# google-research/se3ds

Hardware: AMD Instinct MI355X
Metric: panoramas/sec (G+D train step) at 512x1024 RGB-D (higher is better)
Workload: dtype bf16; 1 GPU; configs/highres 512x1024 full GAN step train_g_d (G+D+hinge+depth+wc losses, clip, Adam, EMA), ResNet-101 gen_dims 128, per-GPU batch 8, d_step_per_g_step 1; per_gpu_batch=8, global_batch=8, parallelism=dp1

## Files before the change

### include/se3ds_hip.h

```cpp
#ifndef SE3DS_HIP_H_
#define SE3DS_HIP_H_

#include <stddef.h>
#include <stdint.h>

#ifdef __cplusplus
extern "C" {
#endif

#define SE3DS_OK 0
#define SE3DS_E_BADSHAPE (-1)
#define SE3DS_E_BADDTYPE (-2)
#define SE3DS_E_WORKSPACE (-3)
#define SE3DS_E_LAUNCH (-4)
#define SE3DS_E_UNSUPPORTED (-5)

#define SE3DS_F32 0
#define SE3DS_I32 1
#define SE3DS_U8 2
#define SE3DS_BF16 3
#define SE3DS_FEAT_BYTE_RANGE 0x100
#define SE3DS_XYZ1_ONES_PRESET 0x200

const char* se3ds_version(void);
// ... 198 lines not shown
                         int c, const float* mean, const float* rstd, int act, float alpha,
                         float* sums, float* dbeta_out, float* dgamma_out, const void* act_mask,
                         void* workspace, size_t workspace_bytes, void* stream);
int se3ds_norm_bwd_apply(const void* dy, const void* y, const void* x, int dtype, int g, int64_t r,
                         int c, const float* mean, const float* rstd, const float* gamma,
                         const float* sums, float count, int act, float alpha, void* dx,
                         void* dres, const void* act_mask, int in_act, float in_alpha,
                         void* stream);
int se3ds_norm_bwd_apply_rows(const void* dy, const void* x, int dtype, int64_t r, int c,
                              const float* mean, const float* rstd, const float* gamma,
                              const float* sums, float count, int act, float alpha, void* dx,
                              void* dres, const void* act_mask, const float* sum_row,
                              const float* out_row, float* colsum_dst, void* workspace,
                              size_t workspace_bytes, void* stream);
int se3ds_norm_bwd_cg_supported(int dtype, int64_t r, int c, int act, int has_mask, int in_act);
size_t se3ds_norm_bwd_cg_workspace_bytes(int c);
int se3ds_norm_bwd_cg_col_rows(int64_t r, int c);
int se3ds_norm_bwd_cg(const void* dy, const void* x, int dtype, int64_t r, int c, const float* mean,
                      const float* rstd, const float* gamma, float count, int act, float alpha,
                      void* dx, void* dres, const void* act_mask, int in_act, float in_alpha,
                      float* dbeta_out, float* dgamma_out, float* sums_out, const float* sum_row,
                      const float* out_row, float* colpart, void* workspace, size_t workspace_bytes,
                      void* stream);
int se3ds_affine_bwd(const void* dy, const void* y, int dtype, int g, int64_t r, int c,
                     const float* scale, int act, float alpha, void* dx, void* dres,
                     const void* act_mask, void* stream);

int se3ds_act_bwd(const void* dy, const void* y, int dtype, int64_t n, int act, float alpha,
                  void* dx, void* stream);
int se3ds_add(const void* a, const void* b, int dtype, int64_t n, void* out, void* stream);
int se3ds_row_scale(const void* x, int dtype, int64_t rows, int c, const float* scale, void* out,
                    void* stream);
int se3ds_maxpool2x2_fwd(const void* x, int dtype, int n, int h, int w, int c, void* y,
                         void* stream);
int se3ds_maxpool2x2_bwd(const void* dy, const void* x, const void* y, int dtype, int n, int h,
                         int w, int c, void* dx, void* stream);
int se3ds_avgpool3s2_fwd(const void* x, int dtype, int n, int h, int w, int c, void* y,
                         void* stream);
int se3ds_avgpool3s2_bwd(const void* dy, int dtype, int n, int h, int w, int c, void* dx,
                         void* stream);
int se3ds_upsample2x_fwd(const void* x, int dtype, int n, int h, int w, int c, void* y,
                         void* stream);
int se3ds_upsample2x_bwd(const void* dy, int dtype, int n, int h, int w, int c, void* dx,
                         void* stream);
int se3ds_copy_channels(const void* src, int src_dtype, int src_c, int src_c0, void* dst,
                        int dst_dtype, int dst_c, int dst_c0, int ncopy, int64_t rows,
// ... 266 lines not shown
```

### se3ds_amd/csrc/norm.hip

```cpp
#include "common.h"
#include <type_traits>
#include <cstdlib>

namespace se3ds {
namespace {

struct Layout2D {
  int cx;
  int ry;
  int vec;
  int ctiles;
};
inline Layout2D make_layout(int C, int V) {
  Layout2D l;
  l.vec = (C % V == 0) ? V : 1;
  int cvec = C / l.vec;
  int cx = 1;
  while (cx < cvec && cx < 256) cx <<= 1;
  l.cx = cx;
  l.ry = 256 / cx;
  l.ctiles = (int)ceil_div(cvec, cx);
  return l;
}

// ... 156 lines not shown
    red2[k][q][ch] = v;
    __syncthreads();
    if (t < 128) {
      const int kk = t >> 6;
      const int c = blockIdx.y * 64 + ch;
      if (c < C)
        partial[(((int64_t)g * rblocks + blockIdx.x) * 2 + kk) * C + c] = (float)(red2[kk][0][ch] + red2[kk][1][ch]);
    }
    return;
  }
  if (ty == 0 && cok) {
    for (int t = 1; t < ry; ++t) {
#pragma unroll
      for (int e = 0; e < VEC; ++e) {
        s0[e] += red[0][(t * cx + tx) * VEC + e];
        s1[e] += red[1][(t * cx + tx) * VEC + e];
      }
    }
    float* P = partial + (((int64_t)g * rblocks + blockIdx.x) * 2) * C;
#pragma unroll
    for (int e = 0; e < VEC; ++e) {
      P[c0 + e] = (float)s0[e];
      P[C + c0 + e] = (float)s1[e];
    }
  }
}

template <int COLS, int LANES>
__global__ void __launch_bounds__(256)
norm_final_reduce_kernel(const float* __restrict__ partial, int rblocks, int C, int G,
                         float* __restrict__ sums, float* __restrict__ dst0,
                         float* __restrict__ dst1) {
  static_assert(COLS * LANES == 256, "block shape");
  __shared__ double sh[LANES][COLS + 1];
  const int g = blockIdx.y;
  const int cl = threadIdx.x % COLS;
  const int col = blockIdx.x * COLS + cl;
  const int lane_b = threadIdx.x / COLS;
  double s0 = 0, s1 = 0, s2 = 0, s3 = 0;
  if (col < 2 * C) {
    const float* P = partial + (int64_t)g * rblocks * 2 * C + col;
    int b = lane_b;
    for (; b + 3 * LANES < rblocks; b += 4 * LANES) {
      s0 += P[(int64_t)b * 2 * C];
      s1 += P[(int64_t)(b + LANES) * 2 * C];
      s2 += P[(int64_t)(b + 2 * LANES) * 2 * C];
// ... 185 lines not shown
  VT<float>::load(shift + (int64_t)g * C + c0, reinterpret_cast<float(&)[4]>(sh[0]));
  VT<float>::load(shift + (int64_t)g * C + c0 + 4, reinterpret_cast<float(&)[4]>(sh[4]));
  for (int64_t r = (int64_t)blockIdx.x * ry + ty; r < R; r += (int64_t)gridDim.x * ry) {
    const int64_t off = ((int64_t)g * R + r) * C + c0;
    float xv[VEC], rv[VEC], o[VEC];
    VT<T>::load(x + off, xv);
    if (HAS_RES) VT<T>::load(res + off, rv);
    unsigned bits = 0;
#pragma unroll
    for (int e = 0; e < VEC; ++e) {
      float v = xv[e] * sc[e] + sh[e];
      if (HAS_RES) v += rv[e];
      if (ACT == 1) v = v > 0.f ? v : 0.f;
      if (ACT == 2) v = v > 0.f ? v : v * alpha;
      o[e] = v;
      const uint16_t hb = f32_to_bf16(v);
      bits |= ((hb & 0x7fffu) != 0 && (hb & 0x8000u) == 0) ? (1u << e) : 0u;
    }
    VT<T>::store(y + off, o);
    if (amask) amask[off >> 3] = (uint8_t)bits;
  }
}

template <typename T, int VEC>
__global__ void __launch_bounds__(256)
norm_bwd_apply_kernel(const T* __restrict__ dy, const T* __restrict__ y, const T* __restrict__ x,
                      const float* __restrict__ mean, const float* __restrict__ rstd,
                      const float* __restrict__ gamma, const float* __restrict__ sums, float count,
                      int64_t R, int C, int cx, int ry, int act, float alpha, T* __restrict__ dx,
                      T* __restrict__ dres, const uint8_t* __restrict__ amask, int in_act,
                      float in_alpha) {
  const int g = blockIdx.z;
  const int tx = threadIdx.x % cx, ty = threadIdx.x / cx;
  const int c0 = (blockIdx.y * cx + tx) * VEC;
  if (c0 >= C) return;
  float gr[VEC], k1[VEC], c0k[VEC];
  const float inv_count = 1.0f / count;
#pragma unroll
  for (int e = 0; e < VEC; ++e) {
    const int64_t gc = (int64_t)g * C + c0 + e;
    const float mu = mean[gc], rs = rstd[gc];
    gr[e] = (gamma ? gamma[c0 + e] : 1.0f) * rs;
    const float s0 = sums[((int64_t)g * 2) * C + c0 + e] * inv_count;
    const float s1 = sums[((int64_t)g * 2 + 1) * C + c0 + e] * inv_count;
    k1[e] = gr[e] * rs * s1;
    c0k[e] = mu * k1[e] - gr[e] * s0;
// ... 180 lines not shown
  if (ROWS) {
    float* red = lds_buf;
#pragma unroll
    for (int e = 0; e < VEC; ++e) red[threadIdx.x * VEC + e] = bsum[e];
    __syncthreads();
    if (PRO) {
      if (threadIdx.x < 64) {
        float t = 0.f;
#pragma unroll 8
        for (int q = 0; q < 32; ++q) t += red[q * 64 + threadIdx.x];
        colpart[(int64_t)blockIdx.x * C + blockIdx.y * 64 + threadIdx.x] = t;
      }
    } else
    if (ty == 0 && live) {
      const int ny = 256 / cx;
      float* row = colpart + (int64_t)blockIdx.x * 2 * C + c0;
#pragma unroll
      for (int e = 0; e < VEC; ++e) {
        float t = 0.f;
        for (int q = 0; q < ny; ++q) t += red[(q * cx + tx) * VEC + e];
        row[e] = t;
        row[C + e] = 0.f;
      }
    }
  }
}

template <typename T, int VEC>
__global__ void __launch_bounds__(256)
affine_bwd_kernel(const T* __restrict__ dy, const T* __restrict__ y,
                  const float* __restrict__ scale, int64_t R, int C, int cx, int ry, int act,
                  float alpha, T* __restrict__ dx, T* __restrict__ dres,
                  const uint8_t* __restrict__ amask) {
  const int g = blockIdx.z;
  const int tx = threadIdx.x % cx, ty = threadIdx.x / cx;
  const int c0 = (blockIdx.y * cx + tx) * VEC;
  if (c0 >= C) return;
  float sc[VEC];
#pragma unroll
  for (int e = 0; e < VEC; ++e) sc[e] = scale[(int64_t)g * C + c0 + e];
  for (int64_t r = (int64_t)blockIdx.x * ry + ty; r < R; r += (int64_t)gridDim.x * ry) {
    const int64_t off = ((int64_t)g * R + r) * C + c0;
    float dv[VEC], yv[VEC], o[VEC], dr[VEC];
    const bool use_mask = VEC == 8 && amask != nullptr;
    unsigned mbits = 0;
    if constexpr (VEC > 1) {
// ... 350 lines not shown
#define LAUNCH_ST(AC)                                                                             \
  hipLaunchKernelGGL((norm_partial_kernel<uint16_t, 8, 1, true, AC, true>), gs, dim3(256), 0, s, A,  \
                     (const uint16_t*)nullptr, X, mean, rstd, (const float*)nullptr, r, c, 8, 32,    \
                     act, alpha, rb, part, (const uint8_t*)act_mask)
  if (act == 0) LAUNCH_ST(0); else if (act == 1) LAUNCH_ST(1); else LAUNCH_ST(2);
#undef LAUNCH_ST
  const dim3 ga((unsigned)cg_apply_blocks(r, c), (unsigned)(c / 64), 1);
#define LAUNCH_AP(AC, IA, RW)                                                                     \
  hipLaunchKernelGGL((norm_bwd_apply_fast_kernel<AC, IA, RW, true>), ga, dim3(256), 0, s, A, X, mean, \
                     rstd, gamma, part, count, r, c, 8, 32, alpha, (uint16_t*)dx, (uint16_t*)dres,     \
                     (const uint8_t*)act_mask, in_alpha, sum_row, out_row, colpart, rb, dbeta_out,     \
                     dgamma_out, sums_out)
  if (rows) {
    if (act == 0) LAUNCH_AP(0, 0, true); else if (act == 1) LAUNCH_AP(1, 0, true); else LAUNCH_AP(2, 0, true);
  } else if (in_act == 0) {
    if (act == 0) LAUNCH_AP(0, 0, false); else if (act == 1) LAUNCH_AP(1, 0, false); else LAUNCH_AP(2, 0, false);
  } else {
    if (act == 0) LAUNCH_AP(0, 2, false); else if (act == 1) LAUNCH_AP(1, 2, false); else LAUNCH_AP(2, 2, false);
  }
#undef LAUNCH_AP
  return check_launch("norm_bwd_cg");
}

int se3ds_affine_bwd(const void* dy, const void* y, int dtype, int g, int64_t r, int c,
                     const float* scale, int act, float alpha, void* dx, void* dres,
                     const void* act_mask, void* stream) {
  if (g <= 0 || r <= 0 || c <= 0) return SE3DS_E_BADSHAPE;
  hipStream_t s = as_stream(stream);
#define LAUNCH_AFF(T, V)                                                                      \
  hipLaunchKernelGGL((affine_bwd_kernel<T, V>), ew_grid(l, r, g), dim3(256), 0, s,            \
                     (const T*)dy, (const T*)y, scale, r, c, l.cx, l.ry, act, alpha, (T*)dx,  \
                     (T*)dres, (const uint8_t*)act_mask)
  if (dtype == SE3DS_F32) {
    Layout2D l = make_layout(c, 4);
    if (l.vec > 1) LAUNCH_AFF(float, 4); else LAUNCH_AFF(float, 1);
  } else if (dtype == SE3DS_BF16) {
    Layout2D l = make_layout(c, 8);
    if (l.vec > 1) LAUNCH_AFF(uint16_t, 8); else LAUNCH_AFF(uint16_t, 1);
  } else {
    return SE3DS_E_BADDTYPE;
  }
#undef LAUNCH_AFF
  return check_launch("affine_bwd");
}

}
// ... 1 lines not shown
```

### se3ds_amd/hipops/nn.py

```python
import math
import threading
from collections import namedtuple
from types import SimpleNamespace
from typing import List, Optional

import numpy as np
import os

import torch
import torch.distributed as dist

from se3ds_amd import _lib

ACT_NONE, ACT_RELU, ACT_LRELU = 0, 1, 2
BN_EPS, BN_MOMENTUM = 1e-3, 0.99
IN_EPS = 1e-3


def _L():
  return _lib.lib()


def _all_reduce_sum(t, group, kind):
  from se3ds_amd.trainers import dist_utils
# ... 1112 lines not shown
    ctx.record(bwd)
  return out


class NormLayer:

  def __init__(self, store: ParamStore, name, c, kind='batch'):
    self.store, self.name, self.c, self.kind = store, name, c, kind
    store.add(name + '/gamma', (c,), ones_init)
    store.add(name + '/beta', (c,), zeros_init)
    if kind == 'batch':
      store.add(name + '/moving_mean', (c,), zeros_init, trainable=False)
      store.add(name + '/moving_variance', (c,), ones_init, trainable=False)
    self._cg_colpart = None


_NORM_DEBUG = {} if os.environ.get('SE3DS_NORM_DEBUG') else None
_FUSED_BN_BWD = os.environ.get('SE3DS_FUSED_BN_BWD', '0') == '1'
_FUSED_ROW_SCALE = os.environ.get('SE3DS_FUSED_ROW_SCALE', '1') != '0'
_NORM_CG = os.environ.get('SE3DS_NORM_CG', '1') != '0'
_CONVT_2X2 = os.environ.get('SE3DS_CONVT_2X2', '1') != '0'
_MASK_CACHE = os.environ.get('SE3DS_MASK_CACHE', '1') != '0'
_DROP_1X1_MASK = os.environ.get('SE3DS_DROP_1X1_MASK', '1') != '0'


def _norm_debug(who, xd, layer):
  if _NORM_DEBUG is not None:
    key = (who, tuple(xd.shape), layer.kind)
    _NORM_DEBUG[key] = _NORM_DEBUG.get(key, 0) + 1


def _norm_stats(ctx, x, layer, g, r, c, use_moving):
  st, L, inst = layer.store, _L(), layer.kind == 'instance'
  scale = torch.empty((g, c), dtype=torch.float32, device=ctx.device)
  shift, mean, rstd = torch.empty_like(scale), torch.empty_like(scale), torch.empty_like(scale)
  count = float(r)
  affine = (st[layer.name + '/gamma'].data_ptr(), st[layer.name + '/beta'].data_ptr(),
            IN_EPS if inst else BN_EPS, BN_MOMENTUM)
  mm = st[layer.name + '/moving_mean'] if not inst else None
  mv = st[layer.name + '/moving_variance'] if not inst else None
  outs = (scale.data_ptr(), shift.data_ptr(), mean.data_ptr(), rstd.data_ptr(), _lib.stream())
  fused = x.col_stats
  fused = fused if fused is not None and not inst and fused.shape[2] == c else None
  if use_moving:
    _chk(L.se3ds_norm_finalize(None, 1.0, g, c, *affine, mm.data_ptr(), mv.data_ptr(), 1, *outs),
         'se3ds_norm_finalize')
# ... 2 lines not shown
                                           mm.data_ptr(), mv.data_ptr(), *outs),
         'se3ds_norm_reduce_rows_finalize')
    x.col_stats = None
  else:
    if fused is not None:
      sums = torch.empty((1, 2, c), dtype=torch.float32, device=ctx.device)
      ws = ctx.ws('norm', L.se3ds_norm_workspace_bytes(max(1, (fused.shape[0] + 511) // 512), c))
      _chk(L.se3ds_norm_reduce_rows(fused.data_ptr(), fused.shape[0], c, sums.data_ptr(),
                                    ws.data_ptr(), ws.numel(), _lib.stream()),
           'se3ds_norm_reduce_rows')
      x.col_stats = None
    else:
      _norm_debug(layer.name, x.data, layer)
      sums = _colsum(ctx, x.data.data_ptr(), ctx.code, r, c, groups=g)
    if not inst and ctx.world > 1:
      ctx.allreduce_sum(sums)
      count = float(r * ctx.world)
    _chk(L.se3ds_norm_finalize(sums.data_ptr(), count, g, c, *affine, _lib.ptr(mm), _lib.ptr(mv), 0,
                               *outs), 'se3ds_norm_finalize')
  return scale, shift, mean, rstd, count


def norm_act(ctx: Ctx, x: Var, layer: NormLayer, act=ACT_NONE, alpha=0.0, res: Var = None,
             post: Var = None, in_act=None) -> Var:
  xd, inst = x.data, layer.kind == 'instance'
  n, h, w, c = xd.shape
  g, r = (n, h * w) if inst else (1, n * h * w)
  use_moving = (not inst) and (not ctx.training or ctx.bn_use_moving)
  scale, shift, mean, rstd, count = _norm_stats(ctx, x, layer, g, r, c, use_moving)
  y = ctx.empty(xd.shape)
  amask = None
  if (ctx.tape is not None and act != ACT_NONE and post is None and c % 8 == 0 and
      xd.dtype == torch.bfloat16):
    amask = torch.empty(xd.numel() // 8, dtype=torch.uint8, device=ctx.device)
  _chk(_L().se3ds_norm_apply(xd.data_ptr(), ctx.code, g, r, c, scale.data_ptr(), shift.data_ptr(),
                             _lib.ptr(res.data if res is not None else None),
                             _lib.ptr(post.data if post is not None else None), act, float(alpha),
                             y.data_ptr(), _lib.ptr(amask), _lib.stream()), 'se3ds_norm_apply')
  out = Var(y)
  if act != ACT_NONE and ctx.act_taps is not None:
    ctx.act_taps[layer.name] = y
  if (ctx.tape is not None and not inst and not use_moving and post is None and c % 8 == 0 and
      xd.dtype == torch.bfloat16 and (act == ACT_NONE or amask is not None)):
    out.bn_src = BnSrc(xd, amask, mean, rstd, act, alpha)
  sync_bwd = (not inst) and ctx.world > 1 and not use_moving
  if ctx.tape is not None:
    sv = SimpleNamespace(ctx=ctx, x=x, out=out, layer=layer, res=res, post=post, act=act,
                         alpha=float(alpha), in_act=in_act, amask=amask, scale=scale, mean=mean,
                         rstd=rstd, gamma=layer.store[layer.name + '/gamma'], count=count, g=g, r=r,
                         c=c, use_moving=use_moving, sync_bwd=sync_bwd)
    ctx.record(lambda: _norm_bwd(sv), sync=sync_bwd)
  return out


def _norm_bwd(sv):
  ctx, out, xd, c, L = sv.ctx, sv.out, sv.x.data, sv.c, _L()
  dy = out.grad
  fused = out.take_bn_stats()
  out.grad = None
  if dy is None:
    if sv.sync_bwd:
      ctx.allreduce_then(torch.zeros((sv.g, 2, c), dtype=torch.float32, device=ctx.device),
                         lambda: None)
    return
  if sv.post is not None:
    raise NotImplementedError
  lim = ctx.batch_limit
  g, shape = sv.g, xd.shape
  if lim is not None and lim < xd.shape[0]:
    assert sv.layer.kind == 'instance' and dy.shape[0] == lim and not ctx.param_grads
    g, shape = lim, (lim,) + tuple(xd.shape[1:])
  ws = ctx.ws('norm', L.se3ds_norm_workspace_bytes(g, c))
  dres = ctx.empty(shape) if sv.res is not None and sv.res.requires_grad else None
  dx = ctx.empty(shape)
  if sv.use_moving:
    _norm_bwd_moving(sv, dy, dx, dres, g, ws)
  elif (_NORM_CG and not sv.sync_bwd and g == 1 and fused is None and lim is None and
        L.se3ds_norm_bwd_cg_supported(ctx.code, sv.r, c, sv.act, 1 if sv.amask is not None else 0,
                                      sv.in_act[0] if sv.in_act else 0)):
    _norm_bwd_cg(sv, dy, dx, dres)
  else:
    _norm_bwd_split(sv, dy, dx, dres, g, ws, fused, lim)


def _norm_deliver(sv, dx, dres, pre_act, scaled=False):
  if pre_act:
    sv.x.grad_pre_act = True
  accumulate(sv.x, dx)
  if scaled:
    sv.x.grad_scaled = sv.x.gver
  if dres is not None:
    accumulate(sv.res, dres)


# ... 43 lines not shown
  if use_rows:
    nrows = int(L.se3ds_norm_bwd_cg_col_rows(r, c))
    colpart = layer._cg_colpart
    if colpart is None or colpart.numel() < nrows * c:
      colpart = layer._cg_colpart = torch.empty(nrows * c, dtype=torch.float32, device=ctx.device)
  gv, pg = layer.store.grad_views, ctx.param_grads
  in_a, in_alpha = sv.in_act or (0, 0.0)
  _chk(L.se3ds_norm_bwd_cg(
      dy.data_ptr(), x.data.data_ptr(), ctx.code, r, c, sv.mean.data_ptr(), sv.rstd.data_ptr(),
      sv.gamma.data_ptr(), sv.count, sv.act, sv.alpha, dx.data_ptr(), _lib.ptr(dres),
      _lib.ptr(sv.amask), in_a, float(in_alpha),
      gv[layer.name + '/beta'].data_ptr() if pg else None,
      gv[layer.name + '/gamma'].data_ptr() if pg else None, None,
      sink.bias_scale.data_ptr() if use_rows else None,
      sink.out_scale.data_ptr() if use_rows else None, _lib.ptr(colpart), cws.data_ptr(),
      cws.numel(), _lib.stream()), 'se3ds_norm_bwd_cg')
  _norm_debug('cg', x.data, layer)
  if use_rows:
    _norm_debug('fused-rows', x.data, layer)
    reduce_or_defer(ctx, (colpart.data_ptr(), nrows, c // 4, sink.bias_grad().data_ptr()))
  _norm_deliver(sv, dx, dres, bool(sv.in_act), scaled=use_rows)


def _norm_bwd_split(sv, dy, dx, dres, g, ws, fused, lim):
  ctx, x, xd, c, L = sv.ctx, sv.x, sv.x.data, sv.c, _L()
  bs = _norm_bwd_sums(sv, dy, g, ws, fused)
  shared = (sv.r, c, sv.mean.data_ptr(), sv.rstd.data_ptr(), sv.gamma.data_ptr(), bs.data_ptr(),
            sv.count, sv.act, sv.alpha, dx.data_ptr(), _lib.ptr(dres), _lib.ptr(sv.amask))

  def finish():
    sink, rc = x.row_sink, -5
    if (sink is not None and _FUSED_ROW_SCALE and ctx.param_grads and g == 1 and not sv.in_act and
        x.grad is None and lim is None and xd.dtype == torch.bfloat16):
      cws = ctx.ws('norm_rows', L.se3ds_norm_workspace_bytes(3, c))
      rc = L.se3ds_norm_bwd_apply_rows(
          dy.data_ptr(), xd.data_ptr(), ctx.code, *shared, sink.bias_scale.data_ptr(),
          sink.out_scale.data_ptr(), sink.bias_grad().data_ptr(), cws.data_ptr(), cws.numel(),
          _lib.stream())
      if rc == 0:
        _norm_debug('fused-rows', xd, sv.layer)
      elif rc not in (-5, -3):
        _chk(rc, 'se3ds_norm_bwd_apply_rows')
    if rc != 0:
      in_a, in_alpha = sv.in_act or (0, 0.0)
      _chk(L.se3ds_norm_bwd_apply(dy.data_ptr(), sv.out.data.data_ptr(), xd.data_ptr(), ctx.code,
                                  g, *shared, in_a, float(in_alpha), _lib.stream()),
# ... 132 lines not shown
```

### se3ds_amd/models/layers.py

```python
from typing import Optional, Tuple

import torch

from se3ds_amd.hipops import nn
from se3ds_amd.hipops.nn import ACT_LRELU, ACT_NONE, ACT_RELU, ConvLayer, Ctx, NormLayer, Var


class PadLayer:

  def __init__(self, padding: int, circular_pad: bool = False, mode='CONSTANT',
               constant_value=0):
    self.padding = padding
    self.circular_pad = circular_pad
    self.mode = mode
    self.constant_value = constant_value

  def wraps(self, training) -> bool:
    return bool(self.circular_pad and not training)

  def __call__(self, inputs: torch.Tensor, training=None) -> torch.Tensor:
    return nn.pad2d(inputs, self.padding, self.wraps(training), self.mode, self.constant_value)


class PartialConv:
# ... 39 lines not shown

  def __call__(self, ctx: Ctx, feature: Var, pad: Optional[PadLayer] = None, act=ACT_NONE,
               alpha=0.0) -> Var:
    p = pad.padding if pad is not None else 0
    wrap = pad.wraps(ctx.training) if pad is not None else False
    return nn.conv2d(ctx, feature, self.conv, pad=p, wrap=wrap, act=act, alpha=alpha)


class Conv2DTranspose:

  def __init__(self, store, name, in_channels, filters, kernel_size, strides=2, use_bias=True):
    self.conv = ConvLayer(store, name, in_channels, filters, kernel_size, strides, 'SAME',
                          use_bias, 'plain', transpose=True)

  def __call__(self, ctx: Ctx, x: Var) -> Var:
    return nn.conv_transpose2d(ctx, x, self.conv)


class SyncBatchNormalization:
  def __init__(self, store, name, channels):
    self.norm = NormLayer(store, name, channels, 'batch')

  def __call__(self, ctx: Ctx, x: Var, act=ACT_NONE, alpha=0.0, res: Var = None,
               in_act=None) -> Var:
    return nn.norm_act(ctx, x, self.norm, act=act, alpha=alpha, res=res, in_act=in_act)


class InstanceNormalization:
  def __init__(self, store, name, channels):
    self.norm = NormLayer(store, name, channels, 'instance')

  def __call__(self, ctx: Ctx, x: Var, act=ACT_NONE, alpha=0.0) -> Var:
    return nn.norm_act(ctx, x, self.norm, act=act, alpha=alpha)


class Bottleneck:

  def __init__(self, store, name, in_channels, filters=128, strides=1, expansion=4,
               downsample=None, circular_pad=False, partial_fn=PartialConv):
    self.conv1 = partial_fn(store, name + '/conv1', in_channels, filters, 1, 1, 'SAME')
    self.bn1 = SyncBatchNormalization(store, name + '/bn1', filters)
    self.pad1 = PadLayer(1, circular_pad=circular_pad)
    self.conv2 = partial_fn(store, name + '/conv2', filters, filters, 3, strides, 'VALID')
    self.bn2 = SyncBatchNormalization(store, name + '/bn2', filters)
    self.conv3 = partial_fn(store, name + '/conv3', filters, expansion * filters, 1, 1, 'SAME')
    self.bn3 = SyncBatchNormalization(store, name + '/bn3', expansion * filters)
    self.downsample = downsample
    if downsample is not None:
      self.ds_norm = SyncBatchNormalization(store, name + '/ds_norm', expansion * filters)

  def __call__(self, ctx: Ctx, x: Var, mask=None):
    out, update_mask = self.conv1(ctx, x, mask)
    out = self.bn1(ctx, out, act=ACT_RELU)
    out, update_mask = self.conv2(ctx, out, update_mask, pad=self.pad1)
    out = self.bn2(ctx, out, act=ACT_RELU)
    out, update_mask = self.conv3(ctx, out, update_mask)
    residual = x
    if self.downsample is not None:
      residual, _ = self.downsample(ctx, x, mask)
      residual = self.ds_norm(ctx, residual)
    out = self.bn3(ctx, out, act=ACT_RELU, res=residual)
    return out, update_mask


class ResStack:

  def __init__(self, store, name, inplanes, planes, blocks, strides=1, expansion=4,
               circular_pad=False, conv_fn=Conv2D):
    partial_fn = PartialSpectralConv if conv_fn is SpectralConv else PartialConv
    downsample = None
    cin = inplanes
    if strides != 1 or inplanes != planes * expansion:
      downsample = partial_fn(store, name + '/downsample', cin, planes * expansion, 1, strides,
                              'SAME', use_bias=False)
    self.blocks = [Bottleneck(store, name + '/block0', cin, planes, strides, expansion, downsample,
                              circular_pad, partial_fn)]
    for i in range(1, blocks):
      self.blocks.append(Bottleneck(store, name + f'/block{i}', planes * expansion, planes,
                                    expansion=expansion, circular_pad=circular_pad,
                                    partial_fn=partial_fn))

  def __call__(self, ctx: Ctx, x: Var, mask=None):
    out, update_mask = self.blocks[0](ctx, x, mask)
    for block in self.blocks[1:]:
# ... 7 lines not shown
               conv_fn=Conv2D):
    self.pad_a = PadLayer(1, circular_pad=circular_pad)
    self.conv_a = conv_fn(store, name + '/conv_a', inplanes, inplanes, 3, 1, 'VALID',
                          use_bias=False)
    self.bn_a = SyncBatchNormalization(store, name + '/bn_a', inplanes)
    self.transposed = upsample is not None and strides != 1
    if self.transposed:
      self.conv_b = Conv2DTranspose(store, name + '/conv_b', inplanes, planes, 3, strides,
                                    use_bias=False)
    else:
      self.pad_b = PadLayer(1, circular_pad=circular_pad)
      self.conv_b = conv_fn(store, name + '/conv_b', inplanes, planes, 3, strides, 'VALID',
                            use_bias=False)
    self.bn_b = SyncBatchNormalization(store, name + '/bn_b', planes)
    self.upsample = upsample

  def __call__(self, ctx: Ctx, x: Var) -> Var:
    out = self.conv_a(ctx, x, pad=self.pad_a)
    out = self.bn_a(ctx, out, act=ACT_RELU)
    if self.transposed:
      out = self.conv_b(ctx, out)
    else:
      out = self.conv_b(ctx, out, pad=self.pad_b)
    residual = x if self.upsample is None else self.upsample(ctx, x)
    return self.bn_b(ctx, out, act=ACT_RELU, res=residual)


class _Upsample:

  def __init__(self, store, name, inplanes, planes, strides, conv_fn):
    if strides != 1:
      self.conv = Conv2DTranspose(store, name + '/conv', inplanes, planes, 2, strides,
                                  use_bias=False)
      self.t = True
    else:
      self.conv = conv_fn(store, name + '/conv', inplanes, planes, 1, 1, 'VALID', use_bias=False)
      self.t = False
    self.bn = SyncBatchNormalization(store, name + '/bn', planes)

  def __call__(self, ctx, x):
    return self.bn(ctx, self.conv(ctx, x))


class ResStackTranspose:

  def __init__(self, store, name, inplanes, planes, blocks, strides=1, circular_pad=False,
               conv_fn=Conv2D):
    upsample = None
    if strides != 1 or inplanes != planes:
      upsample = _Upsample(store, name + '/upsample', inplanes, planes, strides, conv_fn)
    self.block = []
    for i in range(blocks - 1):
      self.block.append(TransBasicBlock(store, name + f'/block{i}', inplanes, inplanes,
                                        circular_pad=circular_pad, conv_fn=conv_fn))
    self.block.append(TransBasicBlock(store, name + f'/block{blocks - 1}', inplanes, planes, strides,
                                      upsample=upsample, circular_pad=circular_pad,
                                      conv_fn=conv_fn))

  def __call__(self, ctx: Ctx, x: Var, mark: Optional[str] = None, group: int = 1) -> Var:
    for i, b in enumerate(self.block):
      if mark is not None and i % group == 0:
        ctx.mark_segment(f'{mark}/blocks{i}')
      x = b(ctx, x)
    return x
# ... 1 lines not shown
```

Baseline: 42.21 panoramas/sec.

## Fuse downsample batchnorm into residual batchnorm apply and backward pass

Adds paired norm kernels so that the downsample/upsample branch's batchnorm is applied inside the main block's bn3/bn_b apply kernel instead of being materialized separately. The backward pass gets a matching pair kernel that computes both input gradients and both beta/gamma gradients from a single read of dy and the mask. This removes one full-tensor write and read of the normalized residual and some kernel launches per downsampling block. In exchange it adds more code paths, an intermediate bf16 rounding that has to match the old numerics, and fallbacks for the multi-GPU and instance-norm cases.

```diff
diff --git a/include/se3ds_hip.h b/include/se3ds_hip.h
--- a/include/se3ds_hip.h
+++ b/include/se3ds_hip.h
@@ -244,6 +244,16 @@
                       float* dbeta_out, float* dgamma_out, float* sums_out, const float* sum_row,
                       const float* out_row, float* colpart, void* workspace, size_t workspace_bytes,
                       void* stream);
+int se3ds_norm_apply_pair(const void* x, int dtype, int64_t r, int c, const float* scale,
+                          const float* shift, const void* x2, const float* scale2,
+                          const float* shift2, int act, float alpha, void* y, void* act_mask,
+                          void* stream);
+int se3ds_norm_bwd_pair(const void* dy, const void* x, const void* x2, int dtype, int64_t r, int c,
+                        const float* mean, const float* rstd, const float* gamma,
+                        const float* mean2, const float* rstd2, const float* gamma2, float count,
+                        void* dx, void* dx2, const void* act_mask, int cg, float* dbeta_out,
+                        float* dgamma_out, float* dbeta2_out, float* dgamma2_out, void* workspace,
+                        size_t workspace_bytes, void* stream);
 int se3ds_affine_bwd(const void* dy, const void* y, int dtype, int g, int64_t r, int c,
                      const float* scale, int act, float alpha, void* dx, void* dres,
                      const void* act_mask, void* stream);
diff --git a/se3ds_amd/csrc/norm.hip b/se3ds_amd/csrc/norm.hip
--- a/se3ds_amd/csrc/norm.hip
+++ b/se3ds_amd/csrc/norm.hip
@@ -202,6 +202,118 @@
     for (int e = 0; e < VEC; ++e) {
       P[c0 + e] = (float)s0[e];
       P[C + c0 + e] = (float)s1[e];
+    }
+  }
+}
+
+template <bool CG>
+__global__ void __launch_bounds__(256)
+norm_pair_partial_kernel(const uint16_t* __restrict__ a, const uint16_t* __restrict__ x,
+                         const uint16_t* __restrict__ x2, const float* __restrict__ mean,
+                         const float* __restrict__ rstd, const float* __restrict__ mean2,
+                         const float* __restrict__ rstd2, int64_t R, int C, int cx, int ry,
+                         int rblocks, float* __restrict__ partial, float* __restrict__ partial2,
+                         const uint8_t* __restrict__ amask) {
+  constexpr int VEC = 8;
+  __shared__ float red[3][256 * VEC];
+  const int tx = threadIdx.x % cx, ty = threadIdx.x / cx;
+  const int c0 = (blockIdx.y * cx + tx) * VEC;
+  const bool cok = c0 < C;
+  float s0[VEC], s1[VEC], s2[VEC];
+#pragma unroll
+  for (int e = 0; e < VEC; ++e) { s0[e] = 0; s1[e] = 0; s2[e] = 0; }
+  float mu[VEC], rs[VEC], mu2[VEC], rs2[VEC];
+  if (cok) {
+#pragma unroll
+    for (int e = 0; e < VEC; ++e) {
+      mu[e] = mean[c0 + e]; rs[e] = rstd[c0 + e];
+      mu2[e] = mean2[c0 + e]; rs2[e] = rstd2[c0 + e];
+    }
+  }
+  const int64_t rows_per_block = ceil_div(R, rblocks);
+  const int64_t r_lo = (int64_t)blockIdx.x * rows_per_block;
+  int64_t r_hi = r_lo + rows_per_block;
+  if (r_hi > R) r_hi = R;
+  if (cok) {
+    constexpr int NR = 4;
+    for (int64_t r = r_lo + ty; r < r_hi; r += (int64_t)NR * ry) {
+      uint4 qa[NR], qx[NR], qz[NR];
+      unsigned mk[NR];
+      bool ok[NR];
+#pragma unroll
+      for (int u = 0; u < NR; ++u) {
+        ok[u] = r + (int64_t)u * ry < r_hi;
+        const int64_t off = (ok[u] ? r + (int64_t)u * ry : r) * C + c0;
+        qa[u] = ld16(a + off);
+        qx[u] = ld16(x + off);
+        qz[u] = ld16(x2 + off);
+        mk[u] = amask[off >> 3];
+      }
+      __builtin_amdgcn_sched_barrier(0);
+#pragma unroll
+      for (int u = 0; u < NR; ++u) {
+        if (!ok[u]) continue;
+        float av[8], xv[8], zv[8];
+        unpack8(qa[u], av);
+        unpack8(qx[u], xv);
+        unpack8(qz[u], zv);
+#pragma unroll
+        for (int e = 0; e < VEC; ++e) {
+          const float d = ((mk[u] >> e) & 1u) ? av[e] : 0.0f;
+          s0[e] += d;
+          s1[e] += d * ((xv[e] - mu[e]) * rs[e]);
+          s2[e] += d * ((zv[e] - mu2[e]) * rs2[e]);
+        }
+      }
+    }
+  }
+#pragma unroll
+  for (int e = 0; e < VEC; ++e) {
+    red[0][threadIdx.x * VEC + e] = s0[e];
+    red[1][threadIdx.x * VEC + e] = s1[e];
+    red[2][threadIdx.x * VEC + e] = s2[e];
+  }
+  __syncthreads();
+  if constexpr (CG) {
+    __shared__ float red2[3][2][64];
+    const int t = threadIdx.x, q = (t >> 6) & 1, ch = t & 63;
+    for (int k = t >> 7; k < 3; k += 2) {
+      float v = 0;
+#pragma unroll
+      for (int i = 0; i < 16; ++i) v += red[k][(q * 16 + i) * 64 + ch];
+      red2[k][q][ch] = v;
+    }
+    __syncthreads();
+    if (t < 192) {
+      const int kk = t >> 6;
+      const int c = blockIdx.y * 64 + ch;
+      if (c < C) {
+        const float v = red2[kk][0][ch] + red2[kk][1][ch];
+        const int64_t row = (int64_t)blockIdx.x * 2 * C + c;
+        if (kk == 0) { partial[row] = v; partial2[row] = v; }
+        else if (kk == 1) partial[row + C] = v;
+        else partial2[row + C] = v;
+      }
+    }
+    return;
+  }
+  if (ty == 0 && cok) {
+    for (int t = 1; t < ry; ++t) {
+#pragma unroll
+      for (int e = 0; e < VEC; ++e) {
+        s0[e] += red[0][(t * cx + tx) * VEC + e];
+        s1[e] += red[1][(t * cx + tx) * VEC + e];
+        s2[e] += red[2][(t * cx + tx) * VEC + e];
+      }
+    }
+    float* P = partial + (int64_t)blockIdx.x * 2 * C;
+    float* P2 = partial2 + (int64_t)blockIdx.x * 2 * C;
+#pragma unroll
+    for (int e = 0; e < VEC; ++e) {
+      P[c0 + e] = s0[e];
+      P[C + c0 + e] = s1[e];
+      P2[c0 + e] = s0[e];
+      P2[C + c0 + e] = s2[e];
     }
   }
 }
@@ -433,6 +545,48 @@
   }
 }
 
+template <int ACT>
+__global__ void __launch_bounds__(256)
+norm_apply_pair_kernel(const uint16_t* __restrict__ x, const float* __restrict__ scale,
+                       const float* __restrict__ shift, const uint16_t* __restrict__ x2,
+                       const float* __restrict__ scale2, const float* __restrict__ shift2, int64_t R,
+                       int C, int cx, int ry, float alpha, uint16_t* __restrict__ y,
+                       uint8_t* __restrict__ amask) {
+  typedef uint16_t T;
+  constexpr int VEC = 8;
+  const int tx = threadIdx.x % cx, ty = threadIdx.x / cx;
+  const int c0 = (blockIdx.y * cx + tx) * VEC;
+  if (c0 >= C) return;
+  float sc[VEC], sh[VEC], sc2[VEC], sh2[VEC];
+  VT<float>::load(scale + c0, reinterpret_cast<float(&)[4]>(sc[0]));
+  VT<float>::load(scale + c0 + 4, reinterpret_cast<float(&)[4]>(sc[4]));
+  VT<float>::load(shift + c0, reinterpret_cast<float(&)[4]>(sh[0]));
+  VT<float>::load(shift + c0 + 4, reinterpret_cast<float(&)[4]>(sh[4]));
+  VT<float>::load(scale2 + c0, reinterpret_cast<float(&)[4]>(sc2[0]));
+  VT<float>::load(scale2 + c0 + 4, reinterpret_cast<float(&)[4]>(sc2[4]));
+  VT<float>::load(shift2 + c0, reinterpret_cast<float(&)[4]>(sh2[0]));
+  VT<float>::load(shift2 + c0 + 4, reinterpret_cast<float(&)[4]>(sh2[4]));
+  for (int64_t r = (int64_t)blockIdx.x * ry + ty; r < R; r += (int64_t)gridDim.x * ry) {
+    const int64_t off = r * C + c0;
+    float xv[VEC], zv[VEC], o[VEC];
+    VT<T>::load(x + off, xv);
+    VT<T>::load(x2 + off, zv);
+    unsigned bits = 0;
+#pragma unroll
+    for (int e = 0; e < VEC; ++e) {
+      const float rv = bf16_to_f32(f32_to_bf16(__fmaf_rn(zv[e], sc2[e], sh2[e])));
+      float v = __fadd_rn(__fmaf_rn(xv[e], sc[e], sh[e]), rv);
+      if (ACT == 1) v = v > 0.f ? v : 0.f;
+      if (ACT == 2) v = v > 0.f ? v : v * alpha;
+      o[e] = v;
+      const uint16_t hb = f32_to_bf16(v);
+      bits |= ((hb & 0x7fffu) != 0 && (hb & 0x8000u) == 0) ? (1u << e) : 0u;
+    }
+    VT<T>::store(y + off, o);
+    if (amask) amask[off >> 3] = (uint8_t)bits;
+  }
+}
+
 template <typename T, int VEC>
 __global__ void __launch_bounds__(256)
 norm_bwd_apply_kernel(const T* __restrict__ dy, const T* __restrict__ y, const T* __restrict__ x,
@@ -659,6 +813,160 @@
         row[e] = t;
         row[C + e] = 0.f;
       }
+    }
+  }
+}
+
+template <bool PRO>
+__global__ void __launch_bounds__(256)
+norm_pair_bwd_apply_kernel(const uint16_t* __restrict__ dy, const uint16_t* __restrict__ x,
+                           const uint16_t* __restrict__ x2, const float* __restrict__ mean,
+                           const float* __restrict__ rstd, const float* __restrict__ gamma,
+                           const float* __restrict__ mean2, const float* __restrict__ rstd2,
+                           const float* __restrict__ gamma2, const float* __restrict__ sums,
+                           const float* __restrict__ sums2, float count, int64_t R, int C, int cx,
+                           int ry, uint16_t* __restrict__ dx, uint16_t* __restrict__ dx2,
+                           const uint8_t* __restrict__ amask, int prows, float* __restrict__ dbeta,
+                           float* __restrict__ dgamma, float* __restrict__ dbeta2,
+                           float* __restrict__ dgamma2) {
+  typedef uint16_t T;
+  constexpr int VEC = 8;
+  const int tx = threadIdx.x % cx, ty = threadIdx.x / cx;
+  const int c0 = (blockIdx.y * cx + tx) * VEC;
+  if (!PRO && c0 >= C) return;
+  const bool live = c0 < C;
+  float gr[VEC], k1[VEC], c0k[VEC], gr2[VEC], k1b[VEC], c0kb[VEC];
+  __shared__ float pro_sums[PRO ? 2 : 1][PRO ? 2 : 1][PRO ? 64 : 1];
+  __shared__ float lds_buf[PRO ? 4096 : 1];
+  if constexpr (PRO) {
+    float (*pro_red)[32][64] = reinterpret_cast<float (*)[32][64]>(lds_buf);
+    for (int p = 0; p < 2; ++p) {
+      const float* S = p ? sums2 : sums;
+      float a0[VEC], a1[VEC];
+#pragma unroll
+      for (int e = 0; e < VEC; ++e) { a0[e] = 0.f; a1[e] = 0.f; }
+      for (int b = ty; b < prows; b += 32) {
+        const float* P = S + (int64_t)b * 2 * C + c0;
+        float v0[VEC], v1[VEC];
+        VT<float>::load(P, reinterpret_cast<float(&)[4]>(v0[0]));
+        VT<float>::load(P + 4, reinterpret_cast<float(&)[4]>(v0[4]));
+        VT<float>::load(P + C, reinterpret_cast<float(&)[4]>(v1[0]));
+        VT<float>::load(P + C + 4, reinterpret_cast<float(&)[4]>(v1[4]));
+#pragma unroll
+        for (int e = 0; e < VEC; ++e) { a0[e] += v0[e]; a1[e] += v1[e]; }
+      }
+#pragma unroll
+      for (int e = 0; e < VEC; ++e) {
+        pro_red[0][ty][tx * VEC + e] = a0[e];
+        pro_red[1][ty][tx * VEC + e] = a1[e];
+      }
+      __syncthreads();
+      if (threadIdx.x < 128) {
+        const int k = threadIdx.x >> 6, ch = threadIdx.x & 63;
+        double t = 0;
+#pragma unroll 8
+        for (int i = 0; i < 32; ++i) t += pro_red[k][i][ch];
+        const float tf = (float)t;
+        pro_sums[p][k][ch] = tf;
+        if (blockIdx.x == 0) {
+          const int c = blockIdx.y * 64 + ch;
+          float* dst = k == 0 ? (p ? dbeta2 : dbeta) : (p ? dgamma2 : dgamma);
+          if (dst) dst[c] = tf;
+        }
+      }
+      __syncthreads();
+    }
+  }
+  {
+    float mu[VEC], rs[VEC], gm[VEC], s0[VEC], s1[VEC];
+    const float inv_count = 1.0f / count;
+    VT<float>::load(mean + c0, reinterpret_cast<float(&)[4]>(mu[0]));
+    VT<float>::load(mean + c0 + 4, reinterpret_cast<float(&)[4]>(mu[4]));
+    VT<float>::load(rstd + c0, reinterpret_cast<float(&)[4]>(rs[0]));
+    VT<float>::load(rstd + c0 + 4, reinterpret_cast<float(&)[4]>(rs[4]));
+    VT<float>::load(gamma + c0, reinterpret_cast<float(&)[4]>(gm[0]));
+    VT<float>::load(gamma + c0 + 4, reinterpret_cast<float(&)[4]>(gm[4]));
+    if constexpr (PRO) {
+#pragma unroll
+      for (int e = 0; e < VEC; ++e) { s0[e] = pro_sums[0][0][tx * VEC + e]; s1[e] = pro_sums[0][1][tx * VEC + e]; }
+    } else {
+      VT<float>::load(sums + c0, reinterpret_cast<float(&)[4]>(s0[0]));
+      VT<float>::load(sums + c0 + 4, reinterpret_cast<float(&)[4]>(s0[4]));
+      VT<float>::load(sums + C + c0, reinterpret_cast<float(&)[4]>(s1[0]));
+      VT<float>::load(sums + C + c0 + 4, reinterpret_cast<float(&)[4]>(s1[4]));
+      if (blockIdx.x == 0 && ty == 0) {
+#pragma unroll
+        for (int e = 0; e < VEC; ++e) {
+          if (dbeta) dbeta[c0 + e] = s0[e];
+          if (dgamma) dgamma[c0 + e] = s1[e];
+        }
+      }
+    }
+#pragma unroll
+    for (int e = 0; e < VEC; ++e) {
+      gr[e] = gm[e] * rs[e];
+      k1[e] = gr[e] * rs[e] * (s1[e] * inv_count);
+      c0k[e] = mu[e] * k1[e] - gr[e] * (s0[e] * inv_count);
+    }
+    VT<float>::load(mean2 + c0, reinterpret_cast<float(&)[4]>(mu[0]));
+    VT<float>::load(mean2 + c0 + 4, reinterpret_cast<float(&)[4]>(mu[4]));
+    VT<float>::load(rstd2 + c0, reinterpret_cast<float(&)[4]>(rs[0]));
+    VT<float>::load(rstd2 + c0 + 4, reinterpret_cast<float(&)[4]>(rs[4]));
+    VT<float>::load(gamma2 + c0, reinterpret_cast<float(&)[4]>(gm[0]));
+    VT<float>::load(gamma2 + c0 + 4, reinterpret_cast<float(&)[4]>(gm[4]));
+    if constexpr (PRO) {
+#pragma unroll
+      for (int e = 0; e < VEC; ++e) { s0[e] = pro_sums[1][0][tx * VEC + e]; s1[e] = pro_sums[1][1][tx * VEC + e]; }
+    } else {
+      VT<float>::load(sums2 + c0, reinterpret_cast<float(&)[4]>(s0[0]));
+      VT<float>::load(sums2 + c0 + 4, reinterpret_cast<float(&)[4]>(s0[4]));
+      VT<float>::load(sums2 + C + c0, reinterpret_cast<float(&)[4]>(s1[0]));
+      VT<float>::load(sums2 + C + c0 + 4, reinterpret_cast<float(&)[4]>(s1[4]));
+      if (blockIdx.x == 0 && ty == 0) {
+#pragma unroll
+        for (int e = 0; e < VEC; ++e) {
+          if (dbeta2) dbeta2[c0 + e] = s0[e];
+          if (dgamma2) dgamma2[c0 + e] = s1[e];
+        }
+      }
+    }
+#pragma unroll
+    for (int e = 0; e < VEC; ++e) {
+      gr2[e] = gm[e] * rs[e];
+      k1b[e] = gr2[e] * rs[e] * (s1[e] * inv_count);
+      c0kb[e] = mu[e] * k1b[e] - gr2[e] * (s0[e] * inv_count);
+    }
+  }
+  const int64_t stride = (int64_t)gridDim.x * ry;
+  for (int64_t r = (int64_t)blockIdx.x * ry + ty; live && r < R; r += 2 * stride) {
+    const bool two = r + stride < R;
+    const int64_t off0 = r * C + c0;
+    const int64_t off1 = two ? off0 + stride * C : off0;
+    float d0[VEC], d1[VEC], x0[VEC], x1[VEC], z0[VEC], z1[VEC], o[VEC], o2[VEC];
+    const uint4 qd0 = ld16(dy + off0), qx0 = ld16(x + off0), qz0 = ld16(x2 + off0);
+    const uint4 qd1 = ld16(dy + off1), qx1 = ld16(x + off1), qz1 = ld16(x2 + off1);
+    const unsigned m0 = amask[off0 >> 3];
+    const unsigned m1 = amask[off1 >> 3];
+    __builtin_amdgcn_sched_barrier(0);
+    unpack8(qd0, d0); unpack8(qx0, x0); unpack8(qz0, z0);
+    unpack8(qd1, d1); unpack8(qx1, x1); unpack8(qz1, z1);
+#pragma unroll
+    for (int e = 0; e < VEC; ++e) {
+      d0[e] = ((m0 >> e) & 1u) ? d0[e] : 0.0f;
+      o[e] = fmaf(gr[e], d0[e], fmaf(-k1[e], x0[e], c0k[e]));
+      o2[e] = fmaf(gr2[e], d0[e], fmaf(-k1b[e], z0[e], c0kb[e]));
+    }
+    VT<T>::store(dx + off0, o);
+    VT<T>::store(dx2 + off0, o2);
+    if (two) {
+#pragma unroll
+      for (int e = 0; e < VEC; ++e) {
+        d1[e] = ((m1 >> e) & 1u) ? d1[e] : 0.0f;
+        o[e] = fmaf(gr[e], d1[e], fmaf(-k1[e], x1[e], c0k[e]));
+        o2[e] = fmaf(gr2[e], d1[e], fmaf(-k1b[e], z1[e], c0kb[e]));
+      }
+      VT<T>::store(dx + off1, o);
+      VT<T>::store(dx2 + off1, o2);
     }
   }
 }
@@ -1055,6 +1363,74 @@
   return check_launch("norm_bwd_cg");
 }
 
+int se3ds_norm_apply_pair(const void* x, int dtype, int64_t r, int c, const float* scale,
+                          const float* shift, const void* x2, const float* scale2,
+                          const float* shift2, int act, float alpha, void* y, void* act_mask,
+                          void* stream) {
+  if (r <= 0 || c <= 0) return SE3DS_E_BADSHAPE;
+  if (dtype != SE3DS_BF16 || (c % 8) != 0 || act < 0 || act > 2 || x2 == nullptr ||
+      scale2 == nullptr || shift2 == nullptr)
+    return SE3DS_E_UNSUPPORTED;
+  hipStream_t s = as_stream(stream);
+  Layout2D l = make_layout(c, 8);
+#define LAUNCH_PAIR(A)                                                                           \
+  hipLaunchKernelGGL((norm_apply_pair_kernel<A>), ew_grid(l, r, 1), dim3(256), 0, s,             \
+                     (const uint16_t*)x, scale, shift, (const uint16_t*)x2, scale2, shift2, r, c, \
+                     l.cx, l.ry, alpha, (uint16_t*)y, (uint8_t*)act_mask)
+  if (act == 0) LAUNCH_PAIR(0); else if (act == 1) LAUNCH_PAIR(1); else LAUNCH_PAIR(2);
+#undef LAUNCH_PAIR
+  return check_launch("norm_apply_pair");
+}
+
+int se3ds_norm_bwd_pair(const void* dy, const void* x, const void* x2, int dtype, int64_t r, int c,
+                        const float* mean, const float* rstd, const float* gamma,
+                        const float* mean2, const float* rstd2, const float* gamma2, float count,
+                        void* dx, void* dx2, const void* act_mask, int cg, float* dbeta_out,
+                        float* dgamma_out, float* dbeta2_out, float* dgamma2_out, void* workspace,
+                        size_t workspace_bytes, void* stream) {
+  if (r <= 0 || c <= 0) return SE3DS_E_BADSHAPE;
+  if (dtype != SE3DS_BF16 || (c % 8) != 0 || gamma == nullptr || gamma2 == nullptr ||
+      act_mask == nullptr || x2 == nullptr || dx2 == nullptr)
+    return SE3DS_E_UNSUPPORTED;
+  if (cg && !se3ds_norm_bwd_cg_supported(dtype, r, c, 1, 1, 0)) return SE3DS_E_UNSUPPORTED;
+  hipStream_t s = as_stream(stream);
+  const uint16_t* A = (const uint16_t*)dy;
+  const uint16_t* X = (const uint16_t*)x;
+  const uint16_t* Z = (const uint16_t*)x2;
+  const uint8_t* M = (const uint8_t*)act_mask;
+  float* part = (float*)workspace;
+  if (cg) {
+    const size_t one = (size_t)kCgMaxRows * 2 * (size_t)c;
+    if (workspace_bytes < sizeof(float) * 2 * one) return SE3DS_E_WORKSPACE;
+    float* part2 = part + one;
+    const int rb = cg_stat_blocks(r, c);
+    hipLaunchKernelGGL((norm_pair_partial_kernel<true>), dim3((unsigned)rb, (unsigned)(c / 64), 1),
+                       dim3(256), 0, s, A, X, Z, mean, rstd, mean2, rstd2, r, c, 8, 32, rb, part,
+                       part2, M);
+    hipLaunchKernelGGL((norm_pair_bwd_apply_kernel<true>),
+                       dim3((unsigned)cg_apply_blocks(r, c), (unsigned)(c / 64), 1), dim3(256), 0, s,
+                       A, X, Z, mean, rstd, gamma, mean2, rstd2, gamma2, part, part2, count, r, c, 8,
+                       32, (uint16_t*)dx, (uint16_t*)dx2, M, rb, dbeta_out, dgamma_out, dbeta2_out,
+                       dgamma2_out);
+  } else {
+    Layout2D l = make_layout(c, 8);
+    const int rb = pick_rblocks(r, l.ry, l.ctiles, 1);
+    const size_t one = (size_t)rb * 2 * (size_t)c;
+    if (workspace_bytes < sizeof(float) * (2 * one + 4 * (size_t)c)) return SE3DS_E_WORKSPACE;
+    float* part2 = part + one;
+    float* sums = part2 + one;
+    hipLaunchKernelGGL((norm_pair_partial_kernel<false>), dim3((unsigned)rb, (unsigned)l.ctiles, 1),
+                       dim3(256), 0, s, A, X, Z, mean, rstd, mean2, rstd2, r, c, l.cx, l.ry, rb,
+                       part, part2, M);
+    launch_final_reduce(s, part, rb, c, 2, sums, nullptr, nullptr);
+    hipLaunchKernelGGL((norm_pair_bwd_apply_kernel<false>), ew_grid(l, r, 1), dim3(256), 0, s, A, X,
+                       Z, mean, rstd, gamma, mean2, rstd2, gamma2, sums, sums + 2 * (size_t)c, count,
+                       r, c, l.cx, l.ry, (uint16_t*)dx, (uint16_t*)dx2, M, 0, dbeta_out, dgamma_out,
+                       dbeta2_out, dgamma2_out);
+  }
+  return check_launch("norm_bwd_pair");
+}
+
 int se3ds_affine_bwd(const void* dy, const void* y, int dtype, int g, int64_t r, int c,
                      const float* scale, int act, float alpha, void* dx, void* dres,
                      const void* act_mask, void* stream) {
diff --git a/se3ds_amd/hipops/nn.py b/se3ds_amd/hipops/nn.py
--- a/se3ds_amd/hipops/nn.py
+++ b/se3ds_amd/hipops/nn.py
@@ -1158,6 +1158,7 @@
 _CONVT_2X2 = os.environ.get('SE3DS_CONVT_2X2', '1') != '0'
 _MASK_CACHE = os.environ.get('SE3DS_MASK_CACHE', '1') != '0'
 _DROP_1X1_MASK = os.environ.get('SE3DS_DROP_1X1_MASK', '1') != '0'
+_NORM_PAIR = True
 
 
 def _norm_debug(who, xd, layer):
@@ -1206,21 +1207,38 @@
 
 
 def norm_act(ctx: Ctx, x: Var, layer: NormLayer, act=ACT_NONE, alpha=0.0, res: Var = None,
-             post: Var = None, in_act=None) -> Var:
+             post: Var = None, in_act=None, res_layer: NormLayer = None) -> Var:
   xd, inst = x.data, layer.kind == 'instance'
   n, h, w, c = xd.shape
   g, r = (n, h * w) if inst else (1, n * h * w)
   use_moving = (not inst) and (not ctx.training or ctx.bn_use_moving)
+  pair = None
+  if res_layer is not None:
+    if (_NORM_PAIR and xd.dtype == torch.bfloat16 and c % 8 == 0 and not inst and post is None and
+        res_layer.kind == 'batch' and ctx.world == 1 and res.data.shape == xd.shape):
+      scale2, shift2, mean2, rstd2, _ = _norm_stats(ctx, res, res_layer, 1, r, c, use_moving)
+      pair = SimpleNamespace(x=res, layer=res_layer, scale=scale2, shift=shift2, mean=mean2,
+                             rstd=rstd2)
+    else:
+      res = norm_act(ctx, res, res_layer)
   scale, shift, mean, rstd, count = _norm_stats(ctx, x, layer, g, r, c, use_moving)
   y = ctx.empty(xd.shape)
   amask = None
   if (ctx.tape is not None and act != ACT_NONE and post is None and c % 8 == 0 and
       xd.dtype == torch.bfloat16):
     amask = torch.empty(xd.numel() // 8, dtype=torch.uint8, device=ctx.device)
-  _chk(_L().se3ds_norm_apply(xd.data_ptr(), ctx.code, g, r, c, scale.data_ptr(), shift.data_ptr(),
-                             _lib.ptr(res.data if res is not None else None),
-                             _lib.ptr(post.data if post is not None else None), act, float(alpha),
-                             y.data_ptr(), _lib.ptr(amask), _lib.stream()), 'se3ds_norm_apply')
+  if pair is not None:
+    _chk(_L().se3ds_norm_apply_pair(xd.data_ptr(), ctx.code, r, c, scale.data_ptr(),
+                                    shift.data_ptr(), res.data.data_ptr(), pair.scale.data_ptr(),
+                                    pair.shift.data_ptr(), act, float(alpha), y.data_ptr(),
+                                    _lib.ptr(amask), _lib.stream()), 'se3ds_norm_apply_pair')
+    _norm_debug('pair', xd, layer)
+    res = Var(res.data)
+  else:
+    _chk(_L().se3ds_norm_apply(xd.data_ptr(), ctx.code, g, r, c, scale.data_ptr(), shift.data_ptr(),
+                               _lib.ptr(res.data if res is not None else None),
+                               _lib.ptr(post.data if post is not None else None), act, float(alpha),
+                               y.data_ptr(), _lib.ptr(amask), _lib.stream()), 'se3ds_norm_apply')
   out = Var(y)
   if act != ACT_NONE and ctx.act_taps is not None:
     ctx.act_taps[layer.name] = y
@@ -1229,10 +1247,18 @@
     out.bn_src = BnSrc(xd, amask, mean, rstd, act, alpha)
   sync_bwd = (not inst) and ctx.world > 1 and not use_moving
   if ctx.tape is not None:
+    if pair is not None:
+      svb = SimpleNamespace(ctx=ctx, x=pair.x, out=res, layer=pair.layer, res=None, post=None,
+                            act=ACT_NONE, alpha=0.0, in_act=None, amask=None, scale=pair.scale,
+                            mean=pair.mean, rstd=pair.rstd,
+                            gamma=pair.layer.store[pair.layer.name + '/gamma'], count=count, g=1,
+                            r=r, c=c, use_moving=use_moving, sync_bwd=False, pair=None)
+      ctx.record(lambda: _norm_bwd(svb))
+      pair.gamma = svb.gamma
     sv = SimpleNamespace(ctx=ctx, x=x, out=out, layer=layer, res=res, post=post, act=act,
                          alpha=float(alpha), in_act=in_act, amask=amask, scale=scale, mean=mean,
                          rstd=rstd, gamma=layer.store[layer.name + '/gamma'], count=count, g=g, r=r,
-                         c=c, use_moving=use_moving, sync_bwd=sync_bwd)
+                         c=c, use_moving=use_moving, sync_bwd=sync_bwd, pair=pair)
     ctx.record(lambda: _norm_bwd(sv), sync=sync_bwd)
   return out
 
@@ -1254,6 +1280,11 @@
   if lim is not None and lim < xd.shape[0]:
     assert sv.layer.kind == 'instance' and dy.shape[0] == lim and not ctx.param_grads
     g, shape = lim, (lim,) + tuple(xd.shape[1:])
+  if (sv.pair is not None and not sv.use_moving and lim is None and fused is None and
+      sv.amask is not None and sv.act == ACT_RELU and not sv.in_act and
+      sv.x.row_sink is None and sv.pair.x.row_sink is None):
+    _norm_bwd_pair(sv, dy)
+    return
   ws = ctx.ws('norm', L.se3ds_norm_workspace_bytes(g, c))
   dres = ctx.empty(shape) if sv.res is not None and sv.res.requires_grad else None
   dx = ctx.empty(shape)
@@ -1343,6 +1374,30 @@
   _norm_deliver(sv, dx, dres, bool(sv.in_act), scaled=use_rows)
 
 
+def _norm_bwd_pair(sv, dy):
+  ctx, x, p, r, c, L = sv.ctx, sv.x, sv.pair, sv.r, sv.c, _L()
+  cg = bool(_NORM_CG and L.se3ds_norm_bwd_cg_supported(ctx.code, r, c, sv.act, 1, 0))
+  ws = ctx.ws('norm_pair', L.se3ds_norm_workspace_bytes(2, c))
+  dx, dx2 = ctx.empty(x.data.shape), ctx.empty(x.data.shape)
+  gv, pg = sv.layer.store.grad_views, ctx.param_grads
+  gv2 = p.layer.store.grad_views
+  _chk(L.se3ds_norm_bwd_pair(
+      dy.data_ptr(), x.data.data_ptr(), p.x.data.data_ptr(), ctx.code, r, c, sv.mean.data_ptr(),
+      sv.rstd.data_ptr(), sv.gamma.data_ptr(), p.mean.data_ptr(), p.rstd.data_ptr(),
+      p.gamma.data_ptr(), sv.count, dx.data_ptr(), dx2.data_ptr(), sv.amask.data_ptr(), int(cg),
+      gv[sv.layer.name + '/beta'].data_ptr() if pg else None,
+      gv[sv.layer.name + '/gamma'].data_ptr() if pg else None,
+      gv2[p.layer.name + '/beta'].data_ptr() if pg else None,
+      gv2[p.layer.name + '/gamma'].data_ptr() if pg else None, ws.data_ptr(), ws.numel(),
+      _lib.stream()), 'se3ds_norm_bwd_pair')
+  _norm_debug('pair-bwd', x.data, sv.layer)
+  if cg:
+    _norm_debug('cg', x.data, sv.layer)
+    _norm_debug('cg', p.x.data, p.layer)
+  accumulate(x, dx)
+  accumulate(p.x, dx2)
+
+
 def _norm_bwd_split(sv, dy, dx, dres, g, ws, fused, lim):
   ctx, x, xd, c, L = sv.ctx, sv.x, sv.x.data, sv.c, _L()
   bs = _norm_bwd_sums(sv, dy, g, ws, fused)
diff --git a/se3ds_amd/models/layers.py b/se3ds_amd/models/layers.py
--- a/se3ds_amd/models/layers.py
+++ b/se3ds_amd/models/layers.py
@@ -85,8 +85,9 @@
     self.norm = NormLayer(store, name, channels, 'batch')
 
   def __call__(self, ctx: Ctx, x: Var, act=ACT_NONE, alpha=0.0, res: Var = None,
-               in_act=None) -> Var:
-    return nn.norm_act(ctx, x, self.norm, act=act, alpha=alpha, res=res, in_act=in_act)
+               in_act=None, res_norm: 'SyncBatchNormalization' = None) -> Var:
+    return nn.norm_act(ctx, x, self.norm, act=act, alpha=alpha, res=res, in_act=in_act,
+                       res_layer=res_norm.norm if res_norm is not None else None)
 
 
 class InstanceNormalization:
@@ -118,11 +119,11 @@
     out, update_mask = self.conv2(ctx, out, update_mask, pad=self.pad1)
     out = self.bn2(ctx, out, act=ACT_RELU)
     out, update_mask = self.conv3(ctx, out, update_mask)
-    residual = x
+    residual, res_norm = x, None
     if self.downsample is not None:
       residual, _ = self.downsample(ctx, x, mask)
-      residual = self.ds_norm(ctx, residual)
-    out = self.bn3(ctx, out, act=ACT_RELU, res=residual)
+      res_norm = self.ds_norm
+    out = self.bn3(ctx, out, act=ACT_RELU, res=residual, res_norm=res_norm)
     return out, update_mask
 
 
@@ -176,8 +177,10 @@
       out = self.conv_b(ctx, out)
     else:
       out = self.conv_b(ctx, out, pad=self.pad_b)
-    residual = x if self.upsample is None else self.upsample(ctx, x)
-    return self.bn_b(ctx, out, act=ACT_RELU, res=residual)
+    if self.upsample is None:
+      return self.bn_b(ctx, out, act=ACT_RELU, res=x)
+    return self.bn_b(ctx, out, act=ACT_RELU, res=self.upsample.conv_only(ctx, x),
+                     res_norm=self.upsample.bn)
 
 
 class _Upsample:
@@ -193,7 +196,10 @@
     self.bn = SyncBatchNormalization(store, name + '/bn', planes)
 
   def __call__(self, ctx, x):
-    return self.bn(ctx, self.conv(ctx, x))
+    return self.bn(ctx, self.conv_only(ctx, x))
+
+  def conv_only(self, ctx, x):
+    return self.conv(ctx, x)
 
 
 class ResStackTranspose:
```

Result: no change. 42.40 panoramas/sec, median of 6 (+0.4%).
